# RobustFieldAutonomyLab/la3dm

Measured on AMD Instinct MI355X. Metric: voxel-updates/sec per scan (200k pts, 0.1 m res); HBM GB/s vs roofline, higher is better.
Workload: dtype f32

## Files before the change

### la3dm_amd/csrc/la3dm_ctx.h

```cpp
#pragma once
#include <hip/hip_runtime.h>

#include <string>
#include <utility>
#include <vector>

#include "../../include/la3dm_hip.h"

struct Arena {
    void *ptr = nullptr;
    size_t cap = 0;
};

struct la3dm_ctx {
    la3dm_params p;
    int device = 0;
    hipStream_t stream = nullptr;
    float4 *d_lut = nullptr;
    uint32_t lut_count = 0;
    std::string err;
    int n_devmaps = 0;
    int opt_bgk_sum = 1;
    int opt_bgk_tables = 1;
    float inv_ell = 0.0f;
    int opt_fast_trig = 0;
    int opt_gp_mode = 0;
    int opt_bgk_tile_desc = 1;
    int opt_grid_order = 0;
    int opt_time_kernel = 0;
    int opt_waves = 1;
    int opt_remap = 2;
    int opt_l_dense_add = 1;
    int opt_l_split_rows = 1024;
    int opt_lds_pad = 0;
    int opt_ablate = 0;
    std::vector<std::pair<hipEvent_t, hipEvent_t>> ev_pool;
    size_t ev_used = 0;
    Arena pts_scaled, nbr_range, blk_desc, label_seq;
    uint32_t scan_seq = 0;
    Arena gp_loff, gp_totals, gp_order, gp_L, gp_alpha, gp_v;
    Arena l_task_item, l_split_list, l_nb_first, l_part, l_counters, l_item_desc, l_rowrec, l_batch_off, l_item_hits, l_bdesc, l_vals, l_rowx, l_dense, l_labmask, l_part64;
    Arena lv_samples, lv_sorted, lv_rays, lv_cell, lv_center, lv_cell0, lv_alpha, lv_beta, lv_state;
    Arena lvp_sub_task, lvp_task, lvp_totals, lvp_rows, lvp_sub_out, lvp_cand;
    Arena h_train, h_train_off, h_nbr, h_center, h_leaf_off, h_leaf_key, h_alpha, h_beta, h_state, h_diag_in,
        h_diag_out;
};

#define HIP_TRY(ctx, expr)                                                                          \
    do {                                                                                            \
        hipError_t e_ = (expr);                                                                     \
        if (e_ != hipSuccess) {                                                                     \
            (ctx)->err = std::string(#expr) + ": " + hipGetErrorString(e_);                          \
            return LA3DM_ERR_HIP;                                                                   \
        }                                                                                           \
    } while (0)

static inline int arena_reserve(la3dm_ctx *ctx, Arena &a, size_t bytes) {
    if (bytes <= a.cap) return LA3DM_OK;
    if (a.ptr) {
        HIP_TRY(ctx, hipFree(a.ptr));
        a.ptr = nullptr;
        a.cap = 0;
    }
    size_t want = bytes + (bytes > (1ull << 30) ? bytes / 8 : bytes / 2) + 256;
    hipError_t e = hipMalloc(&a.ptr, want);
    if (e != hipSuccess) {
        ctx->err = std::string("hipMalloc(") + std::to_string(want) + "): " + hipGetErrorString(e);
        a.ptr = nullptr;
        return LA3DM_ERR_OOM;
    }
    a.cap = want;
    return LA3DM_OK;
}


struct la3dm_lv_pool_scan {
    const float *samples, *sorted, *rays;
    const uint32_t *cell_off;
    int32_t cell_min[3], cell_dim[3];
    uint32_t n_blk;
    const float *blk_center;
    const int32_t *blk_cell0;
    const uint32_t *blk_slot, *blk_mult;
    float *A, *B;
    uint8_t *S;
    uint32_t npb, pass;
    uint32_t *upd_counter;
    uint32_t n_samples;
    uint32_t plan_n_blk;
    const uint32_t *n_blk_dev;
    uint32_t plan_totals[4];
    uint32_t *plan_totals_dev;
};
int la3dm_bgklv_pool_plan_device(la3dm_ctx *ctx, const la3dm_lv_pool_scan *s, uint32_t *totals_dev, hipStream_t stream);
int la3dm_bgklv_pool_scan_device(la3dm_ctx *ctx, const la3dm_lv_pool_scan *s, hipStream_t stream);
```

### la3dm_amd/csrc/la3dm_hip.hip

```cpp
#include "../../include/la3dm_hip.h"

#include <hip/hip_runtime.h>

#include <algorithm>
#include <cmath>
#include <cstdio>
#include <cstdlib>
#include <cstring>
#include <string>
#include <vector>

#include "bgk_kernels.h"
#include "gp_kernels.h"
#include "gp_eigen_kernels.h"
#include "lv_kernels.h"
#include "bgkl_kernels.h"

using namespace la3dm_dev;

#include "la3dm_ctx.h"

static thread_local std::string g_create_error;

static void lv_fill_args(la3dm_ctx *ctx, LvArgs &a, uint32_t n_blk) {
    const int d = ctx->p.block_depth;
    memset(&a, 0, sizeof(a));
    a.lut = ctx->d_lut;
    a.lut_base = 0;
    for (int k = 0; k + 1 < d; ++k) a.lut_base += 1u << (3 * k);
    a.nodes_per_blk = 1u << (3 * (d - 1));
    const uint32_t cubes = (a.nodes_per_blk + kWave - 1) / kWave;
    a.cubes_shift = 0;
    while ((1u << a.cubes_shift) < cubes) ++a.cubes_shift;
    a.cubes_bits = a.cubes_shift / 3;
    a.n_tasks = n_blk << a.cubes_shift;
    const double g = d >= 3 ? 4.0 * (double)ctx->p.resolution : (double)((float)pow(2, d - 1) * ctx->p.resolution);
    a.reach = (int)ceil((double)ctx->p.ell / g);
    a.sf2 = ctx->p.sf2;
    a.ell = ctx->p.ell;
    a.inv_ell = ctx->inv_ell;
    a.free_thresh = ctx->p.free_thresh;
    a.occupied_thresh = ctx->p.occupied_thresh;
    a.var_thresh = ctx->p.var_thresh;
    a.min_W = ctx->p.min_W;
    a.trig = ctx->opt_fast_trig == 3 ? 3 : 0;
}

static uint64_t lv_max_subs(const LvArgs &a, uint32_t n_tasks, uint32_t n_samples) {
    const uint64_t w = 2ull * (uint64_t)a.reach + 1ull, nb = w * w * w;
    return (uint64_t)n_tasks + nb * (uint64_t)n_samples / kLvChunk + 1;
}
static void lv_plan_layout(la3dm_ctx *ctx, LvArgs &a, uint32_t n_tasks, uint32_t n_samples) {
    a.max_subs = (uint32_t)lv_max_subs(a, n_tasks, n_samples);
    a.sub_task = (uint32_t *)ctx->lvp_sub_task.ptr;
    a.task_first = (uint32_t *)ctx->lvp_task.ptr;
    a.task_nsub = a.task_first + n_tasks;
    a.task_row0 = a.task_nsub + n_tasks;
    a.split_list = a.task_row0 + n_tasks;
}
static int lv_plan_launch(la3dm_ctx *ctx, LvArgs &a, uint32_t n_samples, uint32_t *totals_dev, hipStream_t stream, bool zero_totals = true) {
    const uint64_t max_subs = lv_max_subs(a, a.n_tasks, n_samples);
    if (max_subs > 0x3FFFFFFFull) {
        ctx->err = "lv scan: too many cubes x samples for the work plan";
        return LA3DM_ERR_ARG;
    }
    int rc;
    if ((rc = arena_reserve(ctx, ctx->lvp_sub_task, 8 * max_subs)) != LA3DM_OK) return rc;
    if ((rc = arena_reserve(ctx, ctx->lvp_task, 16ull * a.n_tasks)) != LA3DM_OK) return rc;
    if ((rc = arena_reserve(ctx, ctx->lvp_cand, sizeof(LvCand) * (size_t)(n_samples ? n_samples : 1))) != LA3DM_OK) return rc;
    a.cand = (LvCand *)ctx->lvp_cand.ptr;
    a.n_samples = n_samples;
    if (n_samples) hipLaunchKernelGGL(bgklv_cand_kernel, dim3((n_samples + 255) / 256), dim3(256), 0, stream, a);
    lv_plan_layout(ctx, a, a.n_tasks, n_samples);
    a.plan_totals = totals_dev;
    if (zero_totals) HIP_TRY(ctx, hipMemsetAsync(totals_dev, 0, 16, stream));
    hipLaunchKernelGGL(bgklv_plan_kernel, dim3((a.n_tasks + 4 * kLvPlanPerWave - 1) / (4 * kLvPlanPerWave)), dim3(256), 0, stream, a);
    HIP_TRY(ctx, hipGetLastError());
    return LA3DM_OK;
}

static int lv_run_planned(la3dm_ctx *ctx, LvArgs &a, const uint32_t totals[4], hipStream_t stream) {
    const uint32_t n_heavy = totals[0], n_rows = totals[1], n_split = totals[2], n_subs = totals[0] + totals[3];
    if (n_subs == 0) return LA3DM_OK;
    int rc;
    const bool lv_f64 = ctx->opt_bgk_sum == 1;
    if ((rc = arena_reserve(ctx, ctx->lvp_rows, lv_f64 ? sizeof(double2) * kWave * (size_t)(n_heavy ? n_heavy : 1) : 256ull * (n_rows ? n_rows : 1))) != LA3DM_OK) return rc;
    constexpr size_t kWords = kLvChunk / kWave;
    if ((rc = arena_reserve(ctx, ctx->lvp_sub_out, 8ull * (2 * kWords + 1) * n_subs)) != LA3DM_OK) return rc;
    a.rows = (float *)ctx->lvp_rows.ptr;
    a.sub_part = (double2 *)ctx->lvp_rows.ptr;
    a.sub_info = (unsigned long long *)ctx->lvp_sub_out.ptr;
    a.sub_nz = a.sub_info + n_subs;
    a.sub_y = a.sub_nz + kWords * n_subs;
    std::pair<hipEvent_t, hipEvent_t> *ev = nullptr;
    if (ctx->opt_time_kernel) {
        if (ctx->ev_used == ctx->ev_pool.size()) {
            std::pair<hipEvent_t, hipEvent_t> p;
            HIP_TRY(ctx, hipEventCreate(&p.first));
            HIP_TRY(ctx, hipEventCreate(&p.second));
            ctx->ev_pool.push_back(p);
        }
        ev = &ctx->ev_pool[ctx->ev_used++];
        HIP_TRY(ctx, hipEventRecord(ev->first, stream));
    }
    if (ctx->opt_bgk_sum == 1) {
        hipLaunchKernelGGL(bgklv_voxel_kernel_w8, dim3(n_subs), dim3(kLvWaves * kWave), 0, stream, a);
        if (n_split) hipLaunchKernelGGL(bgklv_split_apply64, dim3(n_split), dim3(kWave), 0, stream, a);
    } else {
        hipLaunchKernelGGL(bgklv_voxel_kernel<false>, dim3(n_subs), dim3(kLvWaves * kWave), 0, stream, a);
        if (n_split) hipLaunchKernelGGL(bgklv_split_add_kernel, dim3(n_split), dim3(kLvWaves * kWave), 0, stream, a);
    }
    if (ev) HIP_TRY(ctx, hipEventRecord(ev->second, stream));
    HIP_TRY(ctx, hipGetLastError());
    return LA3DM_OK;
}

static int lv_pool_args(la3dm_ctx *ctx, const la3dm_lv_pool_scan *s, LvArgs &a) {
    if (!ctx || !s) return LA3DM_ERR_ARG;
    if (ctx->p.variant != 2) {
        ctx->err = "la3dm_bgklv_pool_scan: the context was not created with variant = 2 (BGKLVOctoMap)";
        return LA3DM_ERR_ARG;
    }
    lv_fill_args(ctx, a, s->n_blk);
    a.samples = (const float4 *)s->samples;
    a.sorted = (const float4 *)s->sorted;
    a.rays = (const float4 *)s->rays;
    a.cell_off = s->cell_off;
    a.blk_center = s->blk_center;
    a.blk_cell0 = s->blk_cell0;
    a.alpha = s->A;
    a.beta = s->B;
    a.state = s->S;
    for (int i = 0; i < 3; ++i) {
        a.cell_min[i] = s->cell_min[i];
        a.cell_dim[i] = s->cell_dim[i];
    }
    a.blk_slot = s->blk_slot;
    a.blk_mult = s->blk_mult;
    a.upd_counter = s->upd_counter;
    a.npb = s->npb;
    a.layer_off = a.lut_base;
    a.pass = s->pass;
    a.n_blk_dev = s->n_blk_dev;
    return LA3DM_OK;
}

int la3dm_bgklv_pool_plan_device(la3dm_ctx *ctx, const la3dm_lv_pool_scan *s, uint32_t *totals_dev, hipStream_t stream) {
    if (!s || s->n_blk == 0) return LA3DM_OK;
    LvArgs a;
    int rc = lv_pool_args(ctx, s, a);
    if (rc != LA3DM_OK) return rc;
    HIP_TRY(ctx, hipSetDevice(ctx->device));
    return lv_plan_launch(ctx, a, s->n_samples, totals_dev, stream, false);
}

int la3dm_bgklv_pool_scan_device(la3dm_ctx *ctx, const la3dm_lv_pool_scan *s, hipStream_t stream) {
    if (!s || s->n_blk == 0) return LA3DM_OK;
    LvArgs a;
    int rc = lv_pool_args(ctx, s, a);
    if (rc != LA3DM_OK) return rc;
    HIP_TRY(ctx, hipSetDevice(ctx->device));
    lv_plan_layout(ctx, a, (s->plan_n_blk ? s->plan_n_blk : s->n_blk) << a.cubes_shift, s->n_samples);
    a.plan_totals = s->plan_totals_dev;
    a.cand = (LvCand *)ctx->lvp_cand.ptr;
    a.n_samples = s->n_samples;
    return lv_run_planned(ctx, a, s->plan_totals, stream);
}

extern "C" {

int la3dm_device_count(void) {
    int n = 0;
    if (hipGetDeviceCount(&n) != hipSuccess) return 0;
    return n;
}

const char *la3dm_version(void) { return "la3dm_hip 0.1 (gfx950)"; }

const char *la3dm_last_error(const la3dm_ctx *ctx) { return ctx ? ctx->err.c_str() : g_create_error.c_str(); }

int la3dm_create(const la3dm_params *params, la3dm_ctx **out) {
    if (!params || !out) {
        g_create_error = "la3dm_create: null argument";
        return LA3DM_ERR_ARG;
    }
    *out = nullptr;
    if (params->block_depth < 1 || params->block_depth > 6 || !(params->ell > 0.0f) || !params->lut_xyz) {
        g_create_error = "la3dm_create: bad params (block_depth must be 1..6, ell > 0, lut_xyz non-null)";
        return LA3DM_ERR_ARG;
    }
    uint32_t want = 0;
    for (int d = 0; d < params->block_depth; ++d) want += 1u << (3 * d);
    if (params->lut_count != want) {
        g_create_error = "la3dm_create: lut_count must be sum_{d<block_depth} 8^d";
        return LA3DM_ERR_ARG;
    }
    int ndev = 0;
    if (hipGetDeviceCount(&ndev) != hipSuccess || ndev <= 0) {
        g_create_error = "la3dm_create: no HIP device visible (this library has no CPU fallback)";
        return LA3DM_ERR_NODEVICE;
    }
    if (params->device < 0 || params->device >= ndev) {
        g_create_error = "la3dm_create: device ordinal out of range";
        return LA3DM_ERR_ARG;
    }
    la3dm_ctx *ctx = new la3dm_ctx;
    ctx->p = *params;
    ctx->p.lut_xyz = nullptr;
    ctx->device = params->device;
    {
        uint32_t eb;
        memcpy(&eb, &params->ell, 4);
        ctx->inv_ell = (eb & 0x7FFFFFu) != 0x7FFFFFu ? 1.0f / params->ell : 0.0f;
    }
    ctx->lut_count = params->lut_count;
    if (const char *ev = getenv("LA3DM_BGK_SUM")) {
        if (ev[0] == '0' || ev[0] == '1') ctx->opt_bgk_sum = ev[0] - '0';
    }
    if (const char *ev = getenv("LA3DM_BGK_TABLES")) {
        if (ev[0] == '0' || ev[0] == '1') ctx->opt_bgk_tables = ev[0] - '0';
    }
    if (const char *ev = getenv("LA3DM_BGKL_SPLIT_ROWS")) {
        char *end = nullptr;
        const long v = strtol(ev, &end, 10);
        if (end != ev && *end == 0 && v >= -1 && v <= (1 << 24)) ctx->opt_l_split_rows = (int)v;
    }
    if (const char *ev = getenv("LA3DM_GP_MODE")) {
        if (ev[0] == '0' || ev[0] == '1') ctx->opt_gp_mode = ev[0] - '0';
    }
    auto fail = [&](const char *what, hipError_t e) {
        g_create_error = std::string(what) + ": " + hipGetErrorString(e);
        delete ctx;
        return LA3DM_ERR_HIP;
    };
    hipError_t e;
    if ((e = hipSetDevice(ctx->device)) != hipSuccess) return fail("hipSetDevice", e);
    if ((e = hipStreamCreateWithFlags(&ctx->stream, hipStreamNonBlocking)) != hipSuccess)
        return fail("hipStreamCreate", e);
    std::vector<float4> lut4(ctx->lut_count);
    for (uint32_t i = 0; i < ctx->lut_count; ++i)
        lut4[i] = make_float4(params->lut_xyz[3 * i], params->lut_xyz[3 * i + 1], params->lut_xyz[3 * i + 2], 0.0f);
    if ((e = hipMalloc((void **)&ctx->d_lut, sizeof(float4) * ctx->lut_count)) != hipSuccess)
        return fail("hipMalloc(lut)", e);
    if ((e = hipMemcpy(ctx->d_lut, lut4.data(), sizeof(float4) * ctx->lut_count, hipMemcpyHostToDevice)) != hipSuccess)
        return fail("hipMemcpy(lut)", e);
    *out = ctx;
    return LA3DM_OK;
}

void la3dm_destroy(la3dm_ctx *ctx) {
    if (!ctx) return;
    if (ctx->n_devmaps > 0) {
        ctx->err = "la3dm_destroy: destroy the context's la3dm_devmap objects first (context kept alive)";
        fprintf(stderr, "%s\n", ctx->err.c_str());
        return;
    }
    (void)hipSetDevice(ctx->device);
    Arena *all[] = {&ctx->l_task_item, &ctx->l_split_list, &ctx->l_nb_first, &ctx->l_part, &ctx->l_counters, &ctx->l_item_desc, &ctx->l_rowrec, &ctx->l_batch_off, &ctx->l_item_hits, &ctx->l_bdesc, &ctx->l_vals, &ctx->l_rowx, &ctx->l_dense, &ctx->l_labmask, &ctx->l_part64,
                    &ctx->pts_scaled, &ctx->nbr_range, &ctx->blk_desc, &ctx->label_seq, &ctx->gp_loff, &ctx->gp_totals, &ctx->gp_order, &ctx->gp_L, &ctx->gp_alpha, &ctx->gp_v, &ctx->lv_samples, &ctx->lv_sorted, &ctx->lv_rays, &ctx->lv_cell, &ctx->lv_center,
                    &ctx->lv_cell0, &ctx->lv_alpha, &ctx->lv_beta, &ctx->lv_state, &ctx->lvp_sub_task, &ctx->lvp_task, &ctx->lvp_cand, &ctx->lvp_totals, &ctx->lvp_rows, &ctx->lvp_sub_out, &ctx->h_train, &ctx->h_train_off, &ctx->h_nbr, &ctx->h_center, &ctx->h_leaf_off,
                    &ctx->h_leaf_key, &ctx->h_alpha, &ctx->h_beta, &ctx->h_state, &ctx->h_diag_in, &ctx->h_diag_out};
    for (Arena *a : all)
        if (a->ptr) (void)hipFree(a->ptr);
    for (auto &p : ctx->ev_pool) {
        (void)hipEventDestroy(p.first);
        (void)hipEventDestroy(p.second);
    }
    if (ctx->d_lut) (void)hipFree(ctx->d_lut);
    if (ctx->stream) (void)hipStreamDestroy(ctx->stream);
    delete ctx;
}

int la3dm_set_option(la3dm_ctx *ctx, const char *name, int value) {
    if (!ctx || !name) return LA3DM_ERR_ARG;
    auto bad_value = [&](const char *allowed) {
        ctx->err = std::string("la3dm_set_option: ") + name + " must be " + allowed;
        return LA3DM_ERR_ARG;
    };
    if (!strcmp(name, "bgk_sum")) {
        if (value < 0 || value > 1) return bad_value("0 or 1");
        ctx->opt_bgk_sum = value;
        return LA3DM_OK;
    }
    if (!strcmp(name, "bgk_tables")) {
        if (value < 0 || value > 1) return bad_value("0 or 1");
        ctx->opt_bgk_tables = value;
        return LA3DM_OK;
    }
    if (!strcmp(name, "fast_trig")) {
        if (value < 0 || value > 3) return bad_value("0, 1, 2 or 3");
        ctx->opt_fast_trig = value;
        return LA3DM_OK;
    }
    if (!strcmp(name, "waves_per_wg")) {
        if (value != 1 && value != 2 && value != 4) return bad_value("1, 2 or 4");
        ctx->opt_waves = value;
        return LA3DM_OK;
    }
    if (!strcmp(name, "ablate")) {
        if (value < 0 || value > 31) return bad_value("0..31");
        ctx->opt_ablate = value;
        return LA3DM_OK;
    }
    if (!strcmp(name, "lds_pad")) {
        if (value < 0 || value > 32768) return bad_value("0..32768");
        ctx->opt_lds_pad = value;
        return LA3DM_OK;
    }
    if (!strcmp(name, "remap")) {
        if (value < 0 || value > 2) return bad_value("0, 1 or 2");
        ctx->opt_remap = value;
        return LA3DM_OK;
    }
    if (!strcmp(name, "bgk_tile_desc")) {
        if (value < 0 || value > 1) return bad_value("0 or 1");
        ctx->opt_bgk_tile_desc = value;
        return LA3DM_OK;
    }
    if (!strcmp(name, "grid_order")) {
        if (value < 0 || value > 1) return bad_value("0 (ascending cloud index inside a voxel-grid cell) or 1 (what libstdc++'s std::sort on the cell index alone leaves, as pcl::VoxelGrid: verification mode)");
        ctx->opt_grid_order = value;
        return LA3DM_OK;
    }
    if (!strcmp(name, "gp_mode")) {
        if (value < 0 || value > 1) return bad_value("0 (FMA chains in ascending order: the parity configuration) or 1 (Eigen 3.3.7 / SSE2 order, no FMA, pexp)");
        ctx->opt_gp_mode = value;
        return LA3DM_OK;
    }
    if (!strcmp(name, "bgkl_split_rows")) {
        if (value < -1 || value > (1 << 24)) return bad_value("-1 (never split) .. 2^24");
        ctx->opt_l_split_rows = value;
        return LA3DM_OK;
    }
    if (!strcmp(name, "bgkl_dense_add")) {
        if (value < 0 || value > 1) return bad_value("0 or 1");
        ctx->opt_l_dense_add = value;
        return LA3DM_OK;
    }
    if (!strcmp(name, "time_kernel")) {
        ctx->opt_time_kernel = value;
        ctx->ev_used = 0;
        return LA3DM_OK;
    }
    ctx->err = std::string("la3dm_set_option: unknown option ") + name;
    return LA3DM_ERR_ARG;
}

int la3dm_get_option(const la3dm_ctx *ctx, const char *name, int *value) {
    if (!ctx || !name || !value) return LA3DM_ERR_ARG;
    if (!strcmp(name, "bgk_sum")) *value = ctx->opt_bgk_sum;
    else if (!strcmp(name, "bgk_tables")) *value = ctx->opt_bgk_tables;
    else if (!strcmp(name, "fast_trig")) *value = ctx->opt_fast_trig;
    else if (!strcmp(name, "gp_mode")) *value = ctx->opt_gp_mode;
    else if (!strcmp(name, "grid_order")) *value = ctx->opt_grid_order;
    else if (!strcmp(name, "bgk_tile_desc")) *value = ctx->opt_bgk_tile_desc;
    else if (!strcmp(name, "waves_per_wg")) *value = ctx->opt_waves;
    else if (!strcmp(name, "remap")) *value = ctx->opt_remap;
    else return LA3DM_ERR_ARG;
    return LA3DM_OK;
}

static int check_scan(la3dm_ctx *ctx, const la3dm_bgk_scan *s) {
    if (!ctx) return LA3DM_ERR_ARG;
    if (!s) {
        ctx->err = "scan: null";
        return LA3DM_ERR_ARG;
    }
    if (s->n_test_blk == 0) return LA3DM_OK;
    if (!s->nbr || !s->blk_center || !s->leaf_off || !s->leaf_key || !s->alpha || !s->beta || !s->state ||
        !s->train_off || (s->n_train_pts && !s->train_xyzy)) {
        ctx->err = "scan: null array pointer";
        return LA3DM_ERR_ARG;
    }
    return LA3DM_OK;
}

int la3dm_bgk_scan_device(la3dm_ctx *ctx, const la3dm_bgk_scan *s, void *stream_, la3dm_bgk_counters *out) {
    int rc = check_scan(ctx, s);
    if (rc != LA3DM_OK) return rc;
    if (out) memset(out, 0, sizeof(*out));
    if (s->n_test_blk == 0) return LA3DM_OK;
    hipStream_t stream = (hipStream_t)stream_;
    HIP_TRY(ctx, hipSetDevice(ctx->device));

    rc = arena_reserve(ctx, ctx->pts_scaled, sizeof(float4) * (size_t)(s->n_train_pts ? s->n_train_pts : 1));
    if (rc != LA3DM_OK) return rc;
    rc = arena_reserve(ctx, ctx->nbr_range, sizeof(uint2) * 7 * (size_t)s->n_test_blk);
    if (rc != LA3DM_OK) return rc;
    const bool sum_f64 = ctx->opt_bgk_sum == 1;
    uint32_t max_leaves = 1u << (3 * (ctx->p.block_depth - 1));
    uint32_t tpb = (max_leaves + kWave - 1) / kWave;
    uint32_t tpb_shift = 0;
    while ((1u << tpb_shift) < tpb) ++tpb_shift;
    const bool tile_desc = sum_f64 && tpb_shift >= 3 && ctx->opt_bgk_tile_desc && !(s->flags & LA3DM_SCAN_UPDATE_UNGATED) &&
                           ctx->p.ell <= 4.0f * ctx->p.resolution;
    const uint32_t desc_shift = tile_desc ? tpb_shift : 0u;
    if (sum_f64) {
        rc = arena_reserve(ctx, ctx->blk_desc, sizeof(uint32_t) * 16 * ((size_t)s->n_test_blk << desc_shift));
        if (rc != LA3DM_OK) return rc;
        if (!ctx->label_seq.ptr) {
            rc = arena_reserve(ctx, ctx->label_seq, sizeof(uint32_t));
            if (rc != LA3DM_OK) return rc;
            HIP_TRY(ctx, hipMemsetAsync(ctx->label_seq.ptr, 0, sizeof(uint32_t), stream));
            ctx->scan_seq = 0;
        }
        if (++ctx->scan_seq == 0u) ctx->scan_seq = 1u;
    }
    const bool use_tables = sum_f64 && ctx->opt_bgk_tables && ctx->p.block_depth >= 3 && (s->flags & LA3DM_SCAN_LABELS_01) != 0u;
    const bool full_blocks = (s->flags & LA3DM_SCAN_FULL_BLOCKS) != 0u && (uint64_t)s->n_leaf == ((uint64_t)s->n_test_blk << (3 * (ctx->p.block_depth - 1)));
    {
        const uint32_t n_nbr = 7u * s->n_test_blk;
        uint32_t n_thr = s->n_train_pts > n_nbr ? s->n_train_pts : n_nbr;
        BgkDescArgs da;
        da.shift = desc_shift;
        da.depth = (uint32_t)ctx->p.block_depth;
        da.leaf_off = s->leaf_off;
        if (desc_shift && n_thr < (s->n_test_blk << desc_shift)) n_thr = s->n_test_blk << desc_shift;
        dim3 g((n_thr + 255) / 256), b(256);
        const bool want_desc = sum_f64;
        hipLaunchKernelGGL(bgk_prepare, g, b, 0, stream, (const float4 *)s->train_xyzy, (float4 *)ctx->pts_scaled.ptr,
                           s->n_train_pts, ctx->p.ell, s->nbr, s->train_off, sum_f64 ? (uint2 *)nullptr : (uint2 *)ctx->nbr_range.ptr, n_nbr,
                           want_desc ? (uint32_t *)ctx->blk_desc.ptr : (uint32_t *)nullptr,
                           sum_f64 ? (uint32_t *)ctx->label_seq.ptr : (uint32_t *)nullptr, ctx->scan_seq, da);
    }

    BgkArgs a;
    a.pts = (const float4 *)ctx->pts_scaled.ptr;
    a.train_off = s->train_off;
    a.nbr = s->nbr;
    a.blk_center = s->blk_center;
    a.leaf_off = s->leaf_off;
    a.leaf_key = s->leaf_key;
    a.alpha = s->alpha;
    a.beta = s->beta;
    a.state = s->state;
    a.lut = ctx->d_lut;
    a.nbr_range = (const uint2 *)ctx->nbr_range.ptr;
    a.blk_desc = (const uint32_t *)ctx->blk_desc.ptr;
    a.label_seq = (const uint32_t *)ctx->label_seq.ptr;
    a.seq = ctx->scan_seq;
    a.n_test_blk = s->n_test_blk;
    a.tpb_shift = tpb_shift;
    a.desc_shift = desc_shift;
    a.n_tasks = s->n_test_blk << tpb_shift;
    a.flags = s->flags | ((uint32_t)ctx->opt_ablate << 8);
    a.remap = (uint32_t)ctx->opt_remap;
    a.depth = (uint32_t)ctx->p.block_depth;
    a.inv_ell = ctx->inv_ell;
    a.sf2 = ctx->p.sf2;
    a.ell = ctx->p.ell;
    a.free_thresh = ctx->p.free_thresh;
    a.occupied_thresh = ctx->p.occupied_thresh;
    a.var_thresh = ctx->p.var_thresh;
    dim3 grid((a.n_tasks + kWavesPerWG - 1) / kWavesPerWG), block(kWavesPerWG * kWave);
    std::pair<hipEvent_t, hipEvent_t> *ev = nullptr;
    if (ctx->opt_time_kernel) {
        if (ctx->ev_used == ctx->ev_pool.size()) {
            std::pair<hipEvent_t, hipEvent_t> p;
            HIP_TRY(ctx, hipEventCreate(&p.first));
            HIP_TRY(ctx, hipEventCreate(&p.second));
            ctx->ev_pool.push_back(p);
        }
        ev = &ctx->ev_pool[ctx->ev_used++];
        HIP_TRY(ctx, hipEventRecord(ev->first, stream));
    }
#define LAUNCH_BGK(KERNEL, ...)                                                                 \
    switch (ctx->opt_fast_trig) {                                                              \
    case 1: hipLaunchKernelGGL((KERNEL<1 __VA_ARGS__>), grid, block, (size_t)ctx->opt_lds_pad, stream, a); break;     \
    case 2: hipLaunchKernelGGL((KERNEL<2 __VA_ARGS__>), grid, block, (size_t)ctx->opt_lds_pad, stream, a); break;     \
    case 3: hipLaunchKernelGGL((KERNEL<3 __VA_ARGS__>), grid, block, (size_t)ctx->opt_lds_pad, stream, a); break;     \
    default: hipLaunchKernelGGL((KERNEL<0 __VA_ARGS__>), grid, block, (size_t)ctx->opt_lds_pad, stream, a); break;    \
    }
    if (sum_f64) {
        grid = dim3(a.n_tasks);
        block = dim3(kWave);
        if (use_tables) {
            if (full_blocks) {
                LAUNCH_BGK(bgk_predict_fuse_t, , false)
            } else {
                LAUNCH_BGK(bgk_predict_fuse_t)
            }
        } else {
            LAUNCH_BGK(bgk_predict_fuse_r)
        }
    } else {
        const int w = ctx->opt_waves;
        grid = dim3((a.n_tasks + w - 1) / w);
        block = dim3(w * kWave);
        if (w == 4) {
            LAUNCH_BGK(bgk_predict_fuse_v5, , 4)
        } else if (w == 2) {
            LAUNCH_BGK(bgk_predict_fuse_v5, , 2)
        } else {
            LAUNCH_BGK(bgk_predict_fuse_v5, , 1)
        }
    }
#undef LAUNCH_BGK
    if (ev) HIP_TRY(ctx, hipEventRecord(ev->second, stream));
    HIP_TRY(ctx, hipGetLastError());
    if (out) {
        out->n_tiles = a.n_tasks;
        out->scratch_bytes = sizeof(float4) * (size_t)s->n_train_pts;
    }
    return LA3DM_OK;
}

typedef int (*scan_device_fn)(la3dm_ctx *, const la3dm_bgk_scan *, void *, la3dm_bgk_counters *);

static int scan_host_common(la3dm_ctx *ctx, const la3dm_bgk_scan *s, la3dm_bgk_counters *out, scan_device_fn run,
                            size_t row_floats = 4) {
    int rc = check_scan(ctx, s);
    if (rc != LA3DM_OK) return rc;
    if (out) memset(out, 0, sizeof(*out));
    if (s->flags & LA3DM_SCAN_ROWS_PREPARED) {
        ctx->err = "la3dm_*_scan_host: LA3DM_SCAN_ROWS_PREPARED is a flag of la3dm_bgkl_scan_device only (rows of 12 floats already in HBM)";
        return LA3DM_ERR_ARG;
    }
    if (s->n_test_blk == 0) return LA3DM_OK;
    HIP_TRY(ctx, hipSetDevice(ctx->device));
    hipStream_t st = ctx->stream;
    struct Up {
        Arena *a;
        const void *src;
        size_t bytes;
    } ups[] = {
        {&ctx->h_train, s->train_xyzy, sizeof(float) * row_floats * (size_t)s->n_train_pts},
        {&ctx->h_train_off, s->train_off, sizeof(uint32_t) * ((size_t)s->n_train_blk + 1)},
        {&ctx->h_nbr, s->nbr, sizeof(int32_t) * 7 * (size_t)s->n_test_blk},
        {&ctx->h_center, s->blk_center, sizeof(float) * 3 * (size_t)s->n_test_blk},
        {&ctx->h_leaf_off, s->leaf_off, sizeof(uint32_t) * ((size_t)s->n_test_blk + 1)},
        {&ctx->h_leaf_key, s->leaf_key, sizeof(uint32_t) * (size_t)s->n_leaf},
        {&ctx->h_alpha, s->alpha, sizeof(float) * (size_t)s->n_leaf},
        {&ctx->h_beta, s->beta, sizeof(float) * (size_t)s->n_leaf},
    };
    for (auto &u : ups) {
        rc = arena_reserve(ctx, *u.a, u.bytes ? u.bytes : 16);
        if (rc != LA3DM_OK) return rc;
        if (u.bytes) HIP_TRY(ctx, hipMemcpyAsync(u.a->ptr, u.src, u.bytes, hipMemcpyHostToDevice, st));
    }
    rc = arena_reserve(ctx, ctx->h_state, s->n_leaf ? s->n_leaf : 16);
    if (rc != LA3DM_OK) return rc;
    la3dm_bgk_scan d = *s;
    d.train_xyzy = (const float *)ctx->h_train.ptr;
    d.train_off = (const uint32_t *)ctx->h_train_off.ptr;
    d.nbr = (const int32_t *)ctx->h_nbr.ptr;
    d.blk_center = (const float *)ctx->h_center.ptr;
    d.leaf_off = (const uint32_t *)ctx->h_leaf_off.ptr;
    d.leaf_key = (const uint32_t *)ctx->h_leaf_key.ptr;
    d.alpha = (float *)ctx->h_alpha.ptr;
    d.beta = (float *)ctx->h_beta.ptr;
    d.state = (uint8_t *)ctx->h_state.ptr;
    rc = run(ctx, &d, st, out);
    if (rc != LA3DM_OK) return rc;
    if (s->n_leaf) {
        HIP_TRY(ctx, hipMemcpyAsync(s->alpha, d.alpha, sizeof(float) * (size_t)s->n_leaf, hipMemcpyDeviceToHost, st));
        HIP_TRY(ctx, hipMemcpyAsync(s->beta, d.beta, sizeof(float) * (size_t)s->n_leaf, hipMemcpyDeviceToHost, st));
        HIP_TRY(ctx, hipMemcpyAsync(s->state, d.state, (size_t)s->n_leaf, hipMemcpyDeviceToHost, st));
    }
    HIP_TRY(ctx, hipStreamSynchronize(st));
    return LA3DM_OK;
}

int la3dm_bgk_scan_host(la3dm_ctx *ctx, const la3dm_bgk_scan *s, la3dm_bgk_counters *out) {
    return scan_host_common(ctx, s, out, la3dm_bgk_scan_device);
}

int la3dm_gp_scan_device(la3dm_ctx *ctx, const la3dm_bgk_scan *s, void *stream_, la3dm_bgk_counters *out) {
    int rc = check_scan(ctx, s);
    if (rc != LA3DM_OK) return rc;
    if (out) memset(out, 0, sizeof(*out));
    if (s->n_test_blk == 0) return LA3DM_OK;
    if (ctx->p.variant != 1) {
        ctx->err = "la3dm_gp_scan: the context was not created with variant = 1 (GPOctoMap)";
        return LA3DM_ERR_ARG;
    }
    hipStream_t stream = (hipStream_t)stream_;
    HIP_TRY(ctx, hipSetDevice(ctx->device));
    const size_t npts = s->n_train_pts ? s->n_train_pts : 1, nblk = s->n_train_blk ? s->n_train_blk : 1;
    if ((rc = arena_reserve(ctx, ctx->pts_scaled, sizeof(float4) * npts)) != LA3DM_OK) return rc;
    if ((rc = arena_reserve(ctx, ctx->nbr_range, sizeof(uint2) * 7 * (size_t)s->n_test_blk)) != LA3DM_OK) return rc;
    if ((rc = arena_reserve(ctx, ctx->gp_loff, sizeof(unsigned long long) * nblk)) != LA3DM_OK) return rc;
    if ((rc = arena_reserve(ctx, ctx->gp_totals, 32)) != LA3DM_OK) return rc;
    if ((rc = arena_reserve(ctx, ctx->gp_order, sizeof(uint32_t) * nblk)) != LA3DM_OK) return rc;
    if ((rc = arena_reserve(ctx, ctx->gp_alpha, sizeof(float) * npts)) != LA3DM_OK) return rc;
    hipLaunchKernelGGL(gp_factor_offsets, dim3(1), dim3(kGpOffThreads), 0, stream, s->train_off, s->n_train_blk,
                       (unsigned long long *)ctx->gp_loff.ptr, (unsigned long long *)ctx->gp_totals.ptr, (uint32_t *)ctx->gp_order.ptr);
    unsigned long long sum_n2 = s->train_sum_n2;
    uint32_t max_n = s->train_max_n;
    if (sum_n2 == 0 || max_n == 0) {
        unsigned long long tot[2] = {0, 0};
        HIP_TRY(ctx, hipMemcpyAsync(tot, ctx->gp_totals.ptr, 16, hipMemcpyDeviceToHost, stream));
        HIP_TRY(ctx, hipStreamSynchronize(stream));
        sum_n2 = tot[0];
        max_n = (uint32_t)tot[1];
    }
    if ((rc = arena_reserve(ctx, ctx->gp_L, sizeof(float) * (size_t)(sum_n2 ? sum_n2 : 1))) != LA3DM_OK) return rc;

    uint32_t max_leaves = 1u << (3 * (ctx->p.block_depth - 1));
    uint32_t tpb = (max_leaves + kWave - 1) / kWave, tpb_shift = 0;
    while ((1u << tpb_shift) < tpb) ++tpb_shift;
    GpArgs a;
    memset(&a, 0, sizeof(a));
    a.n_test_blk = s->n_test_blk;
    a.tpb_shift = tpb_shift;
    a.n_tasks = s->n_test_blk << tpb_shift;
    a.n_train_blk = s->n_train_blk;
    a.vmax = 0;
    a.vscratch = nullptr;
    if (max_n >= (uint32_t)kGpMfmaMinN && ctx->opt_gp_mode != 1) {
        a.vmax = (max_n + 31u) & ~31u;
        if ((rc = arena_reserve(ctx, ctx->gp_v, sizeof(float) * (size_t)a.n_tasks * a.vmax * kWave)) != LA3DM_OK) return rc;
        a.vscratch = (float *)ctx->gp_v.ptr;
    }
    a.pts = (const float4 *)ctx->pts_scaled.ptr;
    a.train_off = s->train_off;
    a.nbr_range = (const uint2 *)ctx->nbr_range.ptr;
    a.nbr = s->nbr;
    a.l_off = (const unsigned long long *)ctx->gp_loff.ptr;
    a.order = (const uint32_t *)ctx->gp_order.ptr;
    a.totals = (const unsigned long long *)ctx->gp_totals.ptr;
    a.Lmat = (float *)ctx->gp_L.ptr;
    a.alpha_k = (float *)ctx->gp_alpha.ptr;
    a.blk_center = s->blk_center;
    a.leaf_off = s->leaf_off;
    a.leaf_key = s->leaf_key;
    a.m_ivar = s->alpha;
    a.ivar = s->beta;
    a.state = s->state;
    a.lut = ctx->d_lut;
    a.scale = (float)(1.73205 / (double)ctx->p.ell);
    a.sf2 = ctx->p.sf2;
    a.noise = ctx->p.noise;
    a.l = ctx->p.l;
    a.min_ivar = ctx->p.min_ivar;
    a.max_ivar = ctx->p.max_ivar;
    a.min_known_ivar = ctx->p.min_known_ivar;
    a.free_thresh = ctx->p.free_thresh;
    a.occupied_thresh = ctx->p.occupied_thresh;
    {
        const uint32_t n_nbr = 7u * s->n_test_blk;
        const uint32_t n_thr = s->n_train_pts > n_nbr ? s->n_train_pts : n_nbr;
        hipLaunchKernelGGL(gp_prepare, dim3((n_thr + 255) / 256), dim3(256), 0, stream, (const float4 *)s->train_xyzy,
                           (float4 *)ctx->pts_scaled.ptr, s->n_train_pts, a.scale, s->nbr, s->train_off,
                           (uint2 *)ctx->nbr_range.ptr, n_nbr);
    }
    const bool eigen_order = ctx->opt_gp_mode == 1;
    if (eigen_order && max_n > (uint32_t)kGpEigenMaxN) {
        ctx->err = "la3dm_gp_scan: gp_mode 1 (Eigen order on the VALU) takes training blocks of up to " + std::to_string(kGpEigenMaxN) +
                   " points; this scan holds one of " + std::to_string(max_n) + " (block_depth 4 and up belong to the matrix-core path: gp_mode 0)";
        return LA3DM_ERR_ARG;
    }
    if (s->n_train_blk && eigen_order) {
        const uint32_t nn = max_n ? max_n : 1u, n_tiny = nn < (uint32_t)kGpTrainTinyN ? nn : (uint32_t)kGpTrainTinyN;
        hipLaunchKernelGGL(gp_train_eigen_kernel, dim3(s->n_train_blk), dim3(kWave), gp_train_wave_lds(n_tiny), stream, a, 0, (int)n_tiny);
        if (nn > n_tiny)
            hipLaunchKernelGGL(gp_train_eigen_kernel, dim3(s->n_train_blk), dim3(kWave), gp_train_wave_lds(nn), stream, a, (int)n_tiny, (int)nn);
    } else if (s->n_train_blk) {
        const uint32_t nn = max_n < (uint32_t)kGpTrainLdsMaxN ? (max_n ? max_n : 1u) : (uint32_t)kGpTrainLdsMaxN;
        const uint32_t n_tiny = nn < (uint32_t)kGpTrainTinyN ? nn : (uint32_t)kGpTrainTinyN;
        hipLaunchKernelGGL(gp_train_wave_kernel, dim3(s->n_train_blk), dim3(kWave), gp_train_wave_lds(n_tiny), stream, a, 0, (int)n_tiny);
        if (nn > n_tiny)
            hipLaunchKernelGGL(gp_train_wave_kernel, dim3(s->n_train_blk), dim3(kWave), gp_train_wave_lds(nn), stream, a, (int)n_tiny, (int)nn);
        if (max_n > (uint32_t)kGpTrainLdsMaxN)
            hipLaunchKernelGGL(gp_train_kernel, dim3(s->n_train_blk), dim3(kWave), 0, stream, a);
    }
    std::pair<hipEvent_t, hipEvent_t> *ev = nullptr;
    if (ctx->opt_time_kernel) {
        if (ctx->ev_used == ctx->ev_pool.size()) {
            std::pair<hipEvent_t, hipEvent_t> p;
            HIP_TRY(ctx, hipEventCreate(&p.first));
            HIP_TRY(ctx, hipEventCreate(&p.second));
            ctx->ev_pool.push_back(p);
        }
        ev = &ctx->ev_pool[ctx->ev_used++];
        HIP_TRY(ctx, hipEventRecord(ev->first, stream));
    }
    if (eigen_order) {
        hipLaunchKernelGGL(gp_predict_fuse_eigen_kernel, dim3(a.n_tasks), dim3(kWave), (size_t)(max_n ? max_n : 1u) * kWave * sizeof(float), stream, a);
    } else {
        const uint32_t rows = max_n < (uint32_t)kGpLdsRows ? (max_n ? max_n : 1u) : (uint32_t)kGpLdsRows;
        const size_t lds = rows * kWave * sizeof(float);
        int lo = -1;
        for (uint32_t hi : {16u, 32u, (uint32_t)kGpLdsRows}) {
            const uint32_t h = hi < rows ? hi : rows;
            hipLaunchKernelGGL(gp_predict_fuse_small_kernel, dim3(a.n_tasks), dim3(kWave), h * kWave * sizeof(float), stream, a, lo, (int)h);
            lo = (int)h;
            if (h == rows) break;
        }
        if (max_n >= (uint32_t)kGpMfmaMinN)
            hipLaunchKernelGGL(gp_predict_fuse_kernel, dim3(a.n_tasks), dim3(kWave),
                               std::max<size_t>(lds, 3 * 32 * 36 * sizeof(float)) , stream, a);
    }
    if (ev) HIP_TRY(ctx, hipEventRecord(ev->second, stream));
    HIP_TRY(ctx, hipGetLastError());
    if (out) {
        out->n_tiles = a.n_tasks;
        out->scratch_bytes = sizeof(float) * (size_t)sum_n2 + sizeof(float4) * (size_t)s->n_train_pts;
    }
    return LA3DM_OK;
}

int la3dm_gp_scan_host(la3dm_ctx *ctx, const la3dm_bgk_scan *s, la3dm_bgk_counters *out) {
    return scan_host_common(ctx, s, out, la3dm_gp_scan_device);
}

int la3dm_diag_mfma_chain(la3dm_ctx *ctx, const float *A, const float *B, int K, uint32_t *mismatches) {
    if (!ctx || !A || !B || !mismatches || K <= 0 || (K & 1)) return LA3DM_ERR_ARG;
    HIP_TRY(ctx, hipSetDevice(ctx->device));
    float *d = nullptr;
    HIP_TRY(ctx, hipMalloc((void **)&d, sizeof(float) * (64 * (size_t)K + 1)));
    unsigned int *dm = (unsigned int *)(d + 64 * (size_t)K);
    hipError_t e = hipMemcpy(d, A, sizeof(float) * 32 * K, hipMemcpyHostToDevice);
    if (e == hipSuccess) e = hipMemcpy(d + 32 * (size_t)K, B, sizeof(float) * 32 * K, hipMemcpyHostToDevice);
    if (e == hipSuccess) e = hipMemset(dm, 0, 4);
    if (e == hipSuccess) {
        hipLaunchKernelGGL(gp_diag_mfma_chain, dim3(1), dim3(kWave), 0, ctx->stream, d, d + 32 * (size_t)K, K, dm);
        e = hipStreamSynchronize(ctx->stream);
    }
    if (e == hipSuccess) e = hipMemcpy(mismatches, dm, 4, hipMemcpyDeviceToHost);
    (void)hipFree(d);
    if (e != hipSuccess) {
        ctx->err = std::string("la3dm_diag_mfma_chain: ") + hipGetErrorString(e);
        return LA3DM_ERR_HIP;
    }
    return LA3DM_OK;
}

int la3dm_bgklv_scan_device(la3dm_ctx *ctx, const la3dm_lv_scan *s, void *stream_, la3dm_bgk_counters *out) {
    if (!ctx) return LA3DM_ERR_ARG;
    if (!s) {
        ctx->err = "lv scan: null";
        return LA3DM_ERR_ARG;
    }
    if (out) memset(out, 0, sizeof(*out));
    if (s->n_blk == 0) return LA3DM_OK;
    if (ctx->p.variant != 2) {
        ctx->err = "la3dm_bgklv_scan: the context was not created with variant = 2 (BGKLVOctoMap)";
        return LA3DM_ERR_ARG;
    }
    if (!s->sorted || !s->samples || !s->cell_off || !s->blk_center || !s->blk_cell0 || !s->alpha || !s->beta ||
        !s->state || (s->n_rays && !s->rays)) {
        ctx->err = "lv scan: null array pointer";
        return LA3DM_ERR_ARG;
    }
    hipStream_t stream = (hipStream_t)stream_;
    HIP_TRY(ctx, hipSetDevice(ctx->device));
    LvArgs a;
    lv_fill_args(ctx, a, s->n_blk);
    a.samples = (const float4 *)s->samples;
    a.sorted = (const float4 *)s->sorted;
    a.rays = (const float4 *)s->rays;
    a.cell_off = s->cell_off;
    a.blk_center = s->blk_center;
    a.blk_cell0 = s->blk_cell0;
    a.alpha = s->alpha;
    a.beta = s->beta;
    a.state = s->state;
    for (int i = 0; i < 3; ++i) {
        a.cell_min[i] = s->cell_min[i];
        a.cell_dim[i] = s->cell_dim[i];
    }
    int rc = arena_reserve(ctx, ctx->lvp_totals, 16);
    if (rc != LA3DM_OK) return rc;
    if ((rc = lv_plan_launch(ctx, a, s->n_samples, (uint32_t *)ctx->lvp_totals.ptr, stream)) != LA3DM_OK) return rc;
    uint32_t totals[4] = {0, 0, 0, 0};
    HIP_TRY(ctx, hipMemcpyAsync(totals, ctx->lvp_totals.ptr, 16, hipMemcpyDeviceToHost, stream));
    HIP_TRY(ctx, hipStreamSynchronize(stream));
    if ((rc = lv_run_planned(ctx, a, totals, stream)) != LA3DM_OK) return rc;
    if (out) out->n_tiles = totals[0] + totals[3];
    return LA3DM_OK;
}

int la3dm_bgkl_scan_device(la3dm_ctx *ctx, const la3dm_bgk_scan *s, void *stream_, la3dm_bgk_counters *out) {
    int rc = check_scan(ctx, s);
    if (rc != LA3DM_OK) return rc;
    if (out) memset(out, 0, sizeof(*out));
    if (s->n_test_blk == 0) return LA3DM_OK;
    if (ctx->p.variant != 3) {
        ctx->err = "la3dm_bgkl_scan: the context was not created with variant = 3 (BGKLOctoMap)";
        return LA3DM_ERR_ARG;
    }
    hipStream_t stream = (hipStream_t)stream_;
    HIP_TRY(ctx, hipSetDevice(ctx->device));
    const uint32_t max_leaves = 1u << (3 * (ctx->p.block_depth - 1));
    const uint32_t tpb = (max_leaves + kWave - 1) / kWave;
    uint32_t tpb_shift = 0;
    while ((1u << tpb_shift) < tpb) ++tpb_shift;
    BgklArgs a;
    a.rows = s->train_xyzy;
    a.row_off = s->train_off;
    a.nbr = s->nbr;
    a.blk_center = s->blk_center;
    a.leaf_off = s->leaf_off;
    a.leaf_key = s->leaf_key;
    a.alpha = s->alpha;
    a.beta = s->beta;
    a.state = s->state;
    a.lut = ctx->d_lut;
    a.n_test_blk = s->n_test_blk;
    a.tpb_shift = tpb_shift;
    a.n_tasks = s->n_test_blk << tpb_shift;
    a.sf2 = ctx->p.sf2;
    a.ell = ctx->p.ell;
    a.inv_ell = ctx->inv_ell;
    a.trig = ctx->opt_fast_trig == 3 ? 3 : 0;
// ... 223 lines not shown
```

Before: 37.63 billion.

## Add single-launch BGK kernel that skips descriptor prepass for depth-3 full blocks

Adds a new kernel that, for depth-3 full-block label-01 scans, reads neighbour and range data directly with scalar loads and gathers raw training points itself. This removes the separate point-scaling, neighbour-range and block-descriptor prepass launch and its scratch buffers. Points are scaled by 1/ell in-register per chunk instead. The path is on by default, and the per-tile neighbour culling from descriptors is replaced with a per-chunk ballot test, which could cost extra work.

```diff
diff --git a/la3dm_amd/csrc/bgk_scan1_kernels.h b/la3dm_amd/csrc/bgk_scan1_kernels.h
--- /dev/null
+++ b/la3dm_amd/csrc/bgk_scan1_kernels.h
@@ -0,0 +1,240 @@
+#pragma once
+#include "bgk_kernels.h"
+
+namespace la3dm_dev {
+
+template <int kTrig>
+__global__ __launch_bounds__(kWave) __attribute__((amdgpu_waves_per_eu(8, 8))) void bgk_predict_fuse_t1(BgkArgs a) {
+    __shared__ __attribute__((aligned(16))) unsigned char s_lds[5120];
+    const uint32_t task = bgk_task_of_workgroup(a);
+    if (task >= a.n_tasks) return;
+    const uint32_t blk = task >> a.tpb_shift;
+    typedef uint32_t u32x4 __attribute__((ext_vector_type(4)));
+    typedef uint32_t u32x2 __attribute__((ext_vector_type(2)));
+    u32x4 n03;
+    u32x2 n45, lbr;
+    uint32_t n6;
+    float cx, cy, cz;
+    asm("s_load_dwordx2 %[lb], %[lop], 0x0\n"
+        "s_load_dwordx4 %[n03], %[nr], 0x0\n"
+        "s_load_dwordx2 %[n45], %[nr], 0x10\n"
+        "s_load_dword %[n6], %[nr], 0x18\n"
+        "s_load_dword %[cx], %[ctr], 0x0\n"
+        "s_load_dword %[cy], %[ctr], 0x4\n"
+        "s_load_dword %[cz], %[ctr], 0x8\n"
+        "s_waitcnt lgkmcnt(0)\n"
+        : [lb] "=&s"(lbr), [n03] "=&s"(n03), [n45] "=&s"(n45), [n6] "=&s"(n6), [cx] "=&s"(cx), [cy] "=&s"(cy), [cz] "=&s"(cz)
+        : [lop] "s"(a.leaf_off + blk), [nr] "s"(a.nbr + 7 * (size_t)blk), [ctr] "s"(a.blk_center + 3 * (size_t)blk));
+    const uint32_t lb0 = lbr[0];
+    if (lbr[1] - lb0 != 1u << (3u * (a.depth - 1u))) return;
+    uint32_t adj[7], pend[7];
+    {
+        const int32_t tb[7] = {(int32_t)n03[0], (int32_t)n03[1], (int32_t)n03[2], (int32_t)n03[3], (int32_t)n45[0], (int32_t)n45[1], (int32_t)n6};
+        u32x2 r[7];
+        auto pair = [&](int b) { return tb[b] >= 0 ? a.train_off + tb[b] : a.leaf_off + blk; };
+        asm("s_load_dwordx2 %0, %7, 0x0\n"
+            "s_load_dwordx2 %1, %8, 0x0\n"
+            "s_load_dwordx2 %2, %9, 0x0\n"
+            "s_load_dwordx2 %3, %10, 0x0\n"
+            "s_load_dwordx2 %4, %11, 0x0\n"
+            "s_load_dwordx2 %5, %12, 0x0\n"
+            "s_load_dwordx2 %6, %13, 0x0\n"
+            "s_waitcnt lgkmcnt(0)\n"
+            : "=&s"(r[0]), "=&s"(r[1]), "=&s"(r[2]), "=&s"(r[3]), "=&s"(r[4]), "=&s"(r[5]), "=&s"(r[6])
+            : "s"(pair(0)), "s"(pair(1)), "s"(pair(2)), "s"(pair(3)), "s"(pair(4)), "s"(pair(5)), "s"(pair(6)));
+        uint32_t pre = 0;
+#pragma unroll
+        for (int b = 0; b < 7; ++b) {
+            const uint32_t first = tb[b] >= 0 ? r[b][0] : 0u, cnt = tb[b] >= 0 ? r[b][1] - r[b][0] : 0u;
+            adj[b] = first - pre;
+            pre += cnt;
+            pend[b] = pre;
+        }
+    }
+    const uint32_t M = pend[6];
+    WaveLdsT &L = *reinterpret_cast<WaveLdsT *>(s_lds);
+    const uint32_t lane = threadIdx.x;
+    const uint32_t tile = task & ((1u << a.tpb_shift) - 1u);
+    const uint32_t li = lb0 + tile * kWave + lane;
+    const uint32_t n_fine = 1u << (3u * (a.depth - 1u));
+    const uint32_t lut_idx = lut_layer_base(a.depth - 1u) + (n_fine - 1u - tile * kWave) - lane;
+
+    auto gather = [&](uint32_t cb) {
+        uint32_t adjv[7];
+#pragma unroll
+        for (int b = 0; b < 7; ++b) {
+            adjv[b] = adj[b];
+            asm volatile("" : "+v"(adjv[b]));
+        }
+        const uint32_t f = min(cb + lane, M - 1u);
+        uint32_t ad;
+        unsigned long long m1, m2, m3, m4, m5, m6;
+        asm("v_cmp_le_u32 %[m1], %[e0], %[f]\n"
+            "v_cmp_le_u32 %[m2], %[e1], %[f]\n"
+            "v_cmp_le_u32 %[m3], %[e2], %[f]\n"
+            "v_cmp_le_u32 %[m4], %[e3], %[f]\n"
+            "v_cmp_le_u32 %[m5], %[e4], %[f]\n"
+            "v_cmp_le_u32 %[m6], %[e5], %[f]\n"
+            "v_cndmask_b32 %[ad], %[a0], %[a1], %[m1]\n"
+            "v_cndmask_b32 %[ad], %[ad], %[a2], %[m2]\n"
+            "v_cndmask_b32 %[ad], %[ad], %[a3], %[m3]\n"
+            "v_cndmask_b32 %[ad], %[ad], %[a4], %[m4]\n"
+            "v_cndmask_b32 %[ad], %[ad], %[a5], %[m5]\n"
+            "v_cndmask_b32 %[ad], %[ad], %[a6], %[m6]\n"
+            : [ad] "=&v"(ad), [m1] "=&s"(m1), [m2] "=&s"(m2), [m3] "=&s"(m3), [m4] "=&s"(m4), [m5] "=&s"(m5), [m6] "=&s"(m6)
+            : [f] "v"(f), [e0] "s"(pend[0]), [e1] "s"(pend[1]), [e2] "s"(pend[2]), [e3] "s"(pend[3]), [e4] "s"(pend[4]),
+              [e5] "s"(pend[5]), [a0] "v"(adjv[0]), [a1] "v"(adjv[1]), [a2] "v"(adjv[2]), [a3] "v"(adjv[3]), [a4] "v"(adjv[4]),
+              [a5] "v"(adjv[5]), [a6] "v"(adjv[6]));
+        return a.pts[f + ad];
+    };
+#if LA3DM_T_EARLY_AB
+    const float A0 = a.alpha[li], B0 = a.beta[li];
+#endif
+    if (M == 0u) {
+        if (!(a.flags & 1u)) a.state[li] = 0;
+        else {
+            const float A = a.alpha[li], B = a.beta[li];
+            a.state[li] = (uint8_t)(classify(A, B, a) | 0x80u);
+        }
+        return;
+    }
+    float4 pc = gather(0), pn = make_float4(0.0f, 0.0f, 0.0f, 0.0f);
+    if (M > (uint32_t)kWave) pn = gather(kWave);
+
+    const float4 off4 = a.lut[lut_idx];
+    const float xs0 = div_by_ell(off4.x + cx, a.ell, a.inv_ell), ys0 = div_by_ell(off4.y + cy, a.ell, a.inv_ell),
+                zs0 = div_by_ell(off4.z + cz, a.ell, a.inv_ell);
+    L.acc0[lane] = 0.0;
+    L.acc1[lane] = 0.0;
+
+    auto rl = [](float v, int l) { return __int_as_float(__builtin_amdgcn_readlane(__float_as_int(v), l)); };
+    const la3dm_v2f X01 = {rl(xs0, 63), rl(xs0, 59)}, X23 = {rl(xs0, 31), rl(xs0, 27)};
+    const la3dm_v2f Y01 = {rl(ys0, 63), rl(ys0, 61)}, Y23 = {rl(ys0, 47), rl(ys0, 45)};
+    const la3dm_v2f Z01 = {rl(zs0, 63), rl(zs0, 62)}, Z23 = {rl(zs0, 55), rl(zs0, 54)};
+    const uint32_t c6 = lane ^ 63u;
+    const uint32_t ix = ((c6 >> 4) & 2u) | ((c6 >> 2) & 1u), iy = ((c6 >> 3) & 2u) | ((c6 >> 1) & 1u), iz = ((c6 >> 2) & 2u) | (c6 & 1u);
+    const uint32_t tab_base = (uint32_t)(uintptr_t)&L.tab[0][0][0];
+    constexpr uint32_t kRowB = 4u * 16u, kHalfB = 12u * kRowB;
+    static_assert(kTabSlots == 32, "the B loop below walks two halves of 16 slots");
+    const uint32_t ax0 = tab_base + ix * kRowB, ay0 = tab_base + (4u + iy) * kRowB, az0 = tab_base + (8u + iz) * kRowB;
+    const uint32_t ring_base = (uint32_t)(uintptr_t)&L.ring[0];
+    const uint32_t w0 = (uint32_t)(uintptr_t)&L.acc0[0] + 8u * lane;
+    if (w0 & 0x200u) __builtin_trap();
+    static_assert(offsetof(WaveLdsT, acc1) - offsetof(WaveLdsT, acc0) == 512, "c_eval adds 512 to the address of acc0[leaf] for a label-1 pair");
+    const float hit_t = __uint_as_float(kHitTBits);
+    const uint32_t tail_cap = ring_base + 8u * (uint32_t)(kRingT - 4 * kWave);
+    uint32_t tailb = ring_base;
+
+    auto c_eval = [&](uint32_t i) {
+        const uint2 e = L.ring[i];
+        const float kv = cov_sparse_fast<kTrig, true, true>(sqrt_cr(__builtin_fabsf(__uint_as_float(e.x))), a.sf2);
+        const double kd = (double)kv;
+        const uint32_t ad = e.y | ((e.x >> 22) & 0x200u);
+        asm volatile("ds_add_f64 %0, %1\n" : : "v"(ad), "v"(kd) : "memory");
+    };
+    auto c_flush = [&]() {
+        __builtin_amdgcn_fence(__ATOMIC_RELEASE, "wavefront");
+        __builtin_amdgcn_wave_barrier();
+        const uint32_t tail = (tailb - ring_base) >> 3;
+        const uint32_t rem = tail & 63u;
+        if (!(a.flags & 0x100u))
+            for (uint32_t p = rem; p < tail; p += kWave) c_eval(p + lane);
+        tailb = ring_base + 8u * rem;
+        __builtin_amdgcn_fence(__ATOMIC_RELEASE, "wavefront");
+        __builtin_amdgcn_wave_barrier();
+    };
+
+    auto chunk = [&](const float4 &pu, const uint32_t cb) {
+        const float px = div_by_ell(pu.x, a.ell, a.inv_ell), py = div_by_ell(pu.y, a.ell, a.inv_ell), pz = div_by_ell(pu.z, a.ell, a.inv_ell);
+        const la3dm_v2f bx = {px, px}, by = {py, py}, bz = {pz, pz};
+        la3dm_v2f x01 = bx - X01, x23 = bx - X23, y01 = by - Y01, y23 = by - Y23, z01 = bz - Z01, z23 = bz - Z23;
+        x01 *= x01, x23 *= x23, y01 *= y01, y23 *= y23, z01 *= z01, z23 *= z23;
+        const float mx = fminf(fminf(x01.x, x01.y), fminf(x23.x, x23.y));
+        const float my = fminf(fminf(y01.x, y01.y), fminf(y23.x, y23.y));
+        const float mz = fminf(fminf(z01.x, z01.y), fminf(z23.x, z23.y));
+        const bool keep = mx + (my + mz) < hit_t && cb + lane < M;
+        const unsigned long long m = __ballot(keep);
+        if (m == 0ull) return;
+        const float sg = 1.0f - (pu.w + pu.w);
+        const la3dm_v2f s2 = {sg, sg};
+        x01 *= s2, x23 *= s2, y01 *= s2, y23 *= s2, z01 *= s2, z23 *= s2;
+        const uint32_t rank = __builtin_amdgcn_mbcnt_hi((uint32_t)(m >> 32), __builtin_amdgcn_mbcnt_lo((uint32_t)m, 0));
+        const uint32_t n = (uint32_t)__popcll(m);
+        for (uint32_t base = 0; base < n; base += kTabSlots) {
+            const uint32_t nr = min(n - base, (uint32_t)kTabSlots), ngroup = (nr + 3u) >> 2;
+            if (lane < 4u && nr + lane < 4u * ngroup) {
+                float big;
+                asm volatile("v_mov_b32 %0, 0x5e268890" : "=v"(big));
+#pragma unroll
+                for (int r = 0; r < 4; ++r) L.tab[(nr + lane) >> 4][r][(nr + lane) & 15u] = big;
+            }
+            const uint32_t slot = rank - base;
+            if (keep && slot < (uint32_t)kTabSlots) {
+                float(&T)[12][16] = L.tab[slot >> 4];
+                const uint32_t c = slot & 15u;
+                T[0][c] = x01.x, T[1][c] = x01.y, T[2][c] = x23.x, T[3][c] = x23.y;
+                T[4][c] = y01.x, T[5][c] = y01.y, T[6][c] = y23.x, T[7][c] = y23.y;
+                T[8][c] = z01.x, T[9][c] = z01.y, T[10][c] = z23.x, T[11][c] = z23.y;
+            }
+            __builtin_amdgcn_fence(__ATOMIC_RELEASE, "wavefront");
+            __builtin_amdgcn_wave_barrier();
+            if (a.flags & 0x200u) continue;
+            uint32_t aX = ax0, aY = ay0, aZ = az0;
+            for (uint32_t g = 0; g < ngroup; g += 2u) {
+                uint32_t st;
+                float tr;
+                unsigned long long hm0, hm1, hm2, hm3;
+                LA3DM_TP_TRIP("0");
+                if (tailb > tail_cap) c_flush();
+                if (g + 1u < ngroup) {
+                    LA3DM_TP_TRIP("16");
+                    if (tailb > tail_cap) c_flush();
+                }
+                const uint32_t step = g == 2u ? kHalfB - 32u : 32u;
+                aX += step, aY += step, aZ += step;
+            }
+        }
+    };
+
+    for (uint32_t cb = 0;;) {
+        chunk(pc, cb);
+        cb += kWave;
+        if (cb >= M) break;
+        pc = pn;
+        if (cb + kWave < M) pn = gather(cb + kWave);
+    }
+
+    __builtin_amdgcn_fence(__ATOMIC_RELEASE, "wavefront");
+    __builtin_amdgcn_wave_barrier();
+    {
+        const uint32_t tail = (tailb - ring_base) >> 3;
+        if (!(a.flags & 0x100u))
+            for (uint32_t p = 0; p < tail; p += kWave)
+                if (p + lane < tail) c_eval(p + lane);
+    }
+    __builtin_amdgcn_fence(__ATOMIC_RELEASE, "wavefront");
+    __builtin_amdgcn_wave_barrier();
+
+    {
+        const double s0 = L.acc0[lane], s1 = L.acc1[lane];
+        const double K = s0 + s1, Y = s1;
+        uint32_t lw = li;
+        asm volatile("" : "+v"(lw));
+        if (K > 0.0 || (a.flags & 1u) != 0u) {
+#if LA3DM_T_EARLY_AB
+            const float A = (float)((double)A0 + Y);
+            const float B = (float)((double)B0 + (K - Y));
+#else
+            const float A = (float)((double)a.alpha[lw] + Y);
+            const float B = (float)((double)a.beta[lw] + (K - Y));
+#endif
+            a.alpha[lw] = A;
+            a.beta[lw] = B;
+            a.state[lw] = (uint8_t)(classify_fast(A, B, a) | 0x80u);
+        } else {
+            a.state[lw] = 0;
+        }
+    }
+}
+
+}
diff --git a/la3dm_amd/csrc/la3dm_ctx.h b/la3dm_amd/csrc/la3dm_ctx.h
--- a/la3dm_amd/csrc/la3dm_ctx.h
+++ b/la3dm_amd/csrc/la3dm_ctx.h
@@ -22,6 +22,7 @@
     int n_devmaps = 0;
     int opt_bgk_sum = 1;
     int opt_bgk_tables = 1;
+    int opt_bgk_one_launch = 1;
     float inv_ell = 0.0f;
     int opt_fast_trig = 0;
     int opt_gp_mode = 0;
diff --git a/la3dm_amd/csrc/la3dm_hip.hip b/la3dm_amd/csrc/la3dm_hip.hip
--- a/la3dm_amd/csrc/la3dm_hip.hip
+++ b/la3dm_amd/csrc/la3dm_hip.hip
@@ -11,6 +11,7 @@
 #include <vector>
 
 #include "bgk_kernels.h"
+#include "bgk_scan1_kernels.h"
 #include "gp_kernels.h"
 #include "gp_eigen_kernels.h"
 #include "lv_kernels.h"
@@ -220,6 +221,9 @@
     if (const char *ev = getenv("LA3DM_BGK_TABLES")) {
         if (ev[0] == '0' || ev[0] == '1') ctx->opt_bgk_tables = ev[0] - '0';
     }
+    if (const char *ev = getenv("LA3DM_BGK_ONE_LAUNCH")) {
+        if (ev[0] == '0' || ev[0] == '1') ctx->opt_bgk_one_launch = ev[0] - '0';
+    }
     if (const char *ev = getenv("LA3DM_BGKL_SPLIT_ROWS")) {
         char *end = nullptr;
         const long v = strtol(ev, &end, 10);
@@ -287,6 +291,11 @@
         ctx->opt_bgk_tables = value;
         return LA3DM_OK;
     }
+    if (!strcmp(name, "bgk_one_launch")) {
+        if (value < 0 || value > 1) return bad_value("0 or 1");
+        ctx->opt_bgk_one_launch = value;
+        return LA3DM_OK;
+    }
     if (!strcmp(name, "fast_trig")) {
         if (value < 0 || value > 3) return bad_value("0, 1, 2 or 3");
         ctx->opt_fast_trig = value;
@@ -350,6 +359,7 @@
     if (!ctx || !name || !value) return LA3DM_ERR_ARG;
     if (!strcmp(name, "bgk_sum")) *value = ctx->opt_bgk_sum;
     else if (!strcmp(name, "bgk_tables")) *value = ctx->opt_bgk_tables;
+    else if (!strcmp(name, "bgk_one_launch")) *value = ctx->opt_bgk_one_launch;
     else if (!strcmp(name, "fast_trig")) *value = ctx->opt_fast_trig;
     else if (!strcmp(name, "gp_mode")) *value = ctx->opt_gp_mode;
     else if (!strcmp(name, "grid_order")) *value = ctx->opt_grid_order;
@@ -383,11 +393,17 @@
     hipStream_t stream = (hipStream_t)stream_;
     HIP_TRY(ctx, hipSetDevice(ctx->device));
 
-    rc = arena_reserve(ctx, ctx->pts_scaled, sizeof(float4) * (size_t)(s->n_train_pts ? s->n_train_pts : 1));
-    if (rc != LA3DM_OK) return rc;
-    rc = arena_reserve(ctx, ctx->nbr_range, sizeof(uint2) * 7 * (size_t)s->n_test_blk);
-    if (rc != LA3DM_OK) return rc;
     const bool sum_f64 = ctx->opt_bgk_sum == 1;
+    const bool use_tables = sum_f64 && ctx->opt_bgk_tables && ctx->p.block_depth >= 3 && (s->flags & LA3DM_SCAN_LABELS_01) != 0u;
+    const bool full_blocks = (s->flags & LA3DM_SCAN_FULL_BLOCKS) != 0u && (uint64_t)s->n_leaf == ((uint64_t)s->n_test_blk << (3 * (ctx->p.block_depth - 1)));
+    const bool one_launch = use_tables && full_blocks && ctx->p.block_depth == 3 && ctx->opt_bgk_one_launch == 1;
+
+    if (!one_launch) {
+        rc = arena_reserve(ctx, ctx->pts_scaled, sizeof(float4) * (size_t)(s->n_train_pts ? s->n_train_pts : 1));
+        if (rc != LA3DM_OK) return rc;
+        rc = arena_reserve(ctx, ctx->nbr_range, sizeof(uint2) * 7 * (size_t)s->n_test_blk);
+        if (rc != LA3DM_OK) return rc;
+    }
     uint32_t max_leaves = 1u << (3 * (ctx->p.block_depth - 1));
     uint32_t tpb = (max_leaves + kWave - 1) / kWave;
     uint32_t tpb_shift = 0;
@@ -395,7 +411,7 @@
     const bool tile_desc = sum_f64 && tpb_shift >= 3 && ctx->opt_bgk_tile_desc && !(s->flags & LA3DM_SCAN_UPDATE_UNGATED) &&
                            ctx->p.ell <= 4.0f * ctx->p.resolution;
     const uint32_t desc_shift = tile_desc ? tpb_shift : 0u;
-    if (sum_f64) {
+    if (sum_f64 && !one_launch) {
         rc = arena_reserve(ctx, ctx->blk_desc, sizeof(uint32_t) * 16 * ((size_t)s->n_test_blk << desc_shift));
         if (rc != LA3DM_OK) return rc;
         if (!ctx->label_seq.ptr) {
@@ -406,9 +422,7 @@
         }
         if (++ctx->scan_seq == 0u) ctx->scan_seq = 1u;
     }
-    const bool use_tables = sum_f64 && ctx->opt_bgk_tables && ctx->p.block_depth >= 3 && (s->flags & LA3DM_SCAN_LABELS_01) != 0u;
-    const bool full_blocks = (s->flags & LA3DM_SCAN_FULL_BLOCKS) != 0u && (uint64_t)s->n_leaf == ((uint64_t)s->n_test_blk << (3 * (ctx->p.block_depth - 1)));
-    {
+    if (!one_launch) {
         const uint32_t n_nbr = 7u * s->n_test_blk;
         uint32_t n_thr = s->n_train_pts > n_nbr ? s->n_train_pts : n_nbr;
         BgkDescArgs da;
@@ -425,7 +439,7 @@
     }
 
     BgkArgs a;
-    a.pts = (const float4 *)ctx->pts_scaled.ptr;
+    a.pts = one_launch ? (const float4 *)s->train_xyzy : (const float4 *)ctx->pts_scaled.ptr;
     a.train_off = s->train_off;
     a.nbr = s->nbr;
     a.blk_center = s->blk_center;
@@ -474,7 +488,9 @@
     if (sum_f64) {
         grid = dim3(a.n_tasks);
         block = dim3(kWave);
-        if (use_tables) {
+        if (one_launch) {
+            LAUNCH_BGK(bgk_predict_fuse_t1)
+        } else if (use_tables) {
             if (full_blocks) {
                 LAUNCH_BGK(bgk_predict_fuse_t, , false)
             } else {
@@ -500,7 +516,7 @@
     HIP_TRY(ctx, hipGetLastError());
     if (out) {
         out->n_tiles = a.n_tasks;
-        out->scratch_bytes = sizeof(float4) * (size_t)s->n_train_pts;
+        out->scratch_bytes = one_launch ? 0 : sizeof(float4) * (size_t)s->n_train_pts;
     }
     return LA3DM_OK;
 }
```

New measurement: 39.77 billion (median of 6 runs). 1.06x the previous value.
